# Florescence/UNet-Medical-Image-Contour-Segmentation

Hardware: NVIDIA B200
Metric: unet512_train_images_per_sec (higher is better)
Workload: dtype bf16

## Files before the change

### unet-medical-image-contour-segmentation_b200/csrc/common.cuh

```cuda
#pragma once
#include <cuda_bf16.h>
#include <cuda_runtime.h>
#include <stdint.h>
#include <stdio.h>

#include <string>

#include "../../include/unetb200.h"

namespace ub {

void set_error(const char* fmt, ...);
int cuda_fail(cudaError_t e, const char* what);

#define UB_CHECK_ARG(cond, ...)                \
  do {                                         \
    if (!(cond)) {                             \
      ub::set_error(__VA_ARGS__);              \
      return UNETB200_E_INVALID;               \
    }                                          \
  } while (0)

#define UB_LAUNCH_CHECK(what)                              \
  do {                                                     \
    cudaError_t e__ = cudaGetLastError();                  \
    if (e__ != cudaSuccess) return ub::cuda_fail(e__, what); \
  } while (0)

int sm_count();
int set_max_dynamic_smem(const void* func, int bytes, const char* what);

template <typename T>
struct Elem;
template <>
struct Elem<float> {
  static __device__ __forceinline__ float ld(const float* p) { return *p; }
  static __device__ __forceinline__ void st(float* p, float v) { *p = v; }
// ... 20 lines not shown
    v[2 * i + 1] = __uint_as_float(w[i] & 0xffff0000u);
  }
}
__device__ __forceinline__ uint32_t pack_bf16x2(float lo, float hi) {
  __nv_bfloat162 t = __floats2bfloat162_rn(lo, hi);
  return *reinterpret_cast<uint32_t*>(&t);
}
__device__ __forceinline__ void store8(float* p, const float v[8]) {
  *reinterpret_cast<float4*>(p) = make_float4(v[0], v[1], v[2], v[3]);
  *reinterpret_cast<float4*>(p + 4) = make_float4(v[4], v[5], v[6], v[7]);
}
__device__ __forceinline__ void store8(__nv_bfloat16* p, const float v[8]) {
  uint4 r;
  r.x = pack_bf16x2(v[0], v[1]);
  r.y = pack_bf16x2(v[2], v[3]);
  r.z = pack_bf16x2(v[4], v[5]);
  r.w = pack_bf16x2(v[6], v[7]);
  *reinterpret_cast<uint4*>(p) = r;
}

__device__ __forceinline__ float warp_sum(float v) {
#pragma unroll
  for (int o = 16; o > 0; o >>= 1) v += __shfl_xor_sync(0xffffffffu, v, o);
  return v;
}
__device__ __forceinline__ double warp_sum(double v) {
#pragma unroll
  for (int o = 16; o > 0; o >>= 1) v += __shfl_xor_sync(0xffffffffu, v, o);
  return v;
}

inline bool aligned16(const void* p) { return (reinterpret_cast<uintptr_t>(p) & 15) == 0; }

}
```

### unet-medical-image-contour-segmentation_b200/csrc/conv_first.cu

```cuda
#include "gconv.cuh"

namespace ub {

__device__ __forceinline__ void first_decode(const GconvDev& d, int m, int& b, int& i, int& j) {
  j = m % d.Wm;
  const int r = m / d.Wm;
  i = r % d.Hm;
  b = r / d.Hm;
}

template <typename T, int CIN>
__global__ void __launch_bounds__(256)
first_conv_fprop_kernel(GconvDev d, const T* __restrict__ x, const T* __restrict__ wp, T* __restrict__ y,
                        float* __restrict__ stats_ws) {
  constexpr int K = 9 * CIN;
  __shared__ float sstat[2][256];
  __shared__ float sw[CIN == 1 ? 1 : K * 256];
  const int G = d.N >> 3, lanes = 256 / G;
  const int g = threadIdx.x % G, lane = threadIdx.x / G;
  const bool active = lane < lanes;
  for (int i = threadIdx.x; i < 2 * 256; i += 256) (&sstat[0][0])[i] = 0.f;
  float wr[CIN == 1 ? K : 1][8];
  if constexpr (CIN == 1) {
#pragma unroll
// ... 300 lines not shown
      for (int c = 0; c < 3; ++c) { win[0][c] = win[1][c]; win[1][c] = win[2][c]; }
    }
  }
  if (stats_ws) {
    __shared__ float wstat[8][2][64];
    const int warp = threadIdx.x >> 5;
#pragma unroll
    for (int i = 0; i < 8; ++i) {
      float a = s[i], c = q[i];
      a += __shfl_xor_sync(0xffffffffu, a, 8); a += __shfl_xor_sync(0xffffffffu, a, 16);
      c += __shfl_xor_sync(0xffffffffu, c, 8); c += __shfl_xor_sync(0xffffffffu, c, 16);
      if ((threadIdx.x & 31) < 8) { wstat[warp][0][g * 8 + i] = a; wstat[warp][1][g * 8 + i] = c; }
    }
    __syncthreads();
    if (threadIdx.x < 128) {
      const int which = threadIdx.x >> 6, c = threadIdx.x & 63;
      float v = 0.f;
#pragma unroll
      for (int w = 0; w < 8; ++w) v += wstat[w][which][c];
      stats_ws[((long long)blockIdx.x * 2 + which) * 64 + c] = v;
    }
  }
}

template <typename T>
__device__ __forceinline__ float first_halo_elem(const GconvDev& d, const T* __restrict__ x, int b, int i0, int j0, int e) {
  const int r = e / (kFT_W + 2), c = e - r * (kFT_W + 2);
  const int gi = i0 - 1 + r, gj = j0 - 1 + c;
  if (e < (kFT_H + 2) * (kFT_W + 2) && (unsigned)gi < (unsigned)d.Hin && (unsigned)gj < (unsigned)d.Win)
    return Elem<T>::ld(x + ((long long)(b * d.Hin + gi) * d.Win + gj) * d.ld_in);
  return 0.f;
}

template <typename T>
__global__ void __launch_bounds__(256, 2)
first_conv_wgrad_tiled_kernel(GconvDev d, const T* __restrict__ x, const T* __restrict__ gy, float* __restrict__ partials,
                              int tiles_w, int tiles_h, int ntiles) {
  __shared__ float halo[kFT_H + 2][kFT_LD];
  const int g = threadIdx.x & 7, pl = threadIdx.x >> 3;
  float acc[3][3][8];
#pragma unroll
  for (int a = 0; a < 3; ++a)
#pragma unroll
    for (int c = 0; c < 3; ++c)
#pragma unroll
      for (int i = 0; i < 8; ++i) acc[a][c][i] = 0.f;
  auto decode = [&](int tile, int& b, int& i0, int& j0) {
    const int tj = tile % tiles_w;
    const int rest = tile / tiles_w;
    b = rest / tiles_h;
    i0 = (rest % tiles_h) * kFT_H;
    j0 = tj * kFT_W;
  };
  struct Row { uint4 a, b; };
  auto load_half = [&](int tile, int half, Row* dst) {
    int b, i0, j0;
    decode(tile, b, i0, j0);
    const int j = j0 + pl;
#pragma unroll
    for (int rr = 0; rr < 4; ++rr) {
      const int i = i0 + half * 4 + rr;
      dst[rr].a = make_uint4(0u, 0u, 0u, 0u);
      dst[rr].b = make_uint4(0u, 0u, 0u, 0u);
      if (tile < ntiles && i < d.Hm && j < d.Wm) {
        const T* src = gy + ((long long)(b * d.Hm + i) * d.Wm + j) * d.ld_out + g * 8;
        dst[rr].a = *reinterpret_cast<const uint4*>(src);
        if constexpr (sizeof(T) == 4) dst[rr].b = *reinterpret_cast<const uint4*>(src + 4);
// ... 2 lines not shown
  };
  auto unpack = [&](const Row& r, float v[8]) {
    if constexpr (sizeof(T) == 4) {
      v[0] = __uint_as_float(r.a.x); v[1] = __uint_as_float(r.a.y); v[2] = __uint_as_float(r.a.z); v[3] = __uint_as_float(r.a.w);
      v[4] = __uint_as_float(r.b.x); v[5] = __uint_as_float(r.b.y); v[6] = __uint_as_float(r.b.z); v[7] = __uint_as_float(r.b.w);
    } else {
      const uint32_t w[4] = {r.a.x, r.a.y, r.a.z, r.a.w};
#pragma unroll
      for (int i = 0; i < 4; ++i) { v[2 * i] = __uint_as_float(w[i] << 16); v[2 * i + 1] = __uint_as_float(w[i] & 0xffff0000u); }
    }
  };
  int tile = blockIdx.x;
  float h0 = 0.f, h1 = 0.f;
  Row cur[4], nxt[4];
  if (tile < ntiles) {
    int b, i0, j0;
    decode(tile, b, i0, j0);
    h0 = first_halo_elem<T>(d, x, b, i0, j0, threadIdx.x);
    h1 = first_halo_elem<T>(d, x, b, i0, j0, threadIdx.x + 256);
  }
  load_half(tile, 0, cur);
  for (; tile < ntiles; tile += gridDim.x) {
    __syncthreads();
    (&halo[0][0])[(threadIdx.x / (kFT_W + 2)) * kFT_LD + threadIdx.x % (kFT_W + 2)] = h0;
    if (threadIdx.x + 256 < (kFT_H + 2) * (kFT_W + 2))
      (&halo[0][0])[((threadIdx.x + 256) / (kFT_W + 2)) * kFT_LD + (threadIdx.x + 256) % (kFT_W + 2)] = h1;
    __syncthreads();
    const int nxt_tile = tile + gridDim.x;
    if (nxt_tile < ntiles) {
      int nb, ni0, nj0;
      decode(nxt_tile, nb, ni0, nj0);
      h0 = first_halo_elem<T>(d, x, nb, ni0, nj0, threadIdx.x);
      h1 = first_halo_elem<T>(d, x, nb, ni0, nj0, threadIdx.x + 256);
    }
    float win[3][3];
#pragma unroll
    for (int a = 0; a < 2; ++a)
#pragma unroll
      for (int c = 0; c < 3; ++c) win[a][c] = halo[a][pl + c];
#pragma unroll
    for (int half = 0; half < 2; ++half) {
      if (half == 0) load_half(tile, 1, nxt); else load_half(nxt_tile, 0, nxt);
#pragma unroll
      for (int rr = 0; rr < 4; ++rr) {
        const int r = half * 4 + rr;
        float gv[8];
        unpack(cur[rr], gv);
#pragma unroll
        for (int c = 0; c < 3; ++c) win[2][c] = halo[r + 2][pl + c];
#pragma unroll
        for (int a = 0; a < 3; ++a)
#pragma unroll
          for (int c = 0; c < 3; ++c)
#pragma unroll
            for (int k = 0; k < 8; ++k) acc[a][c][k] = fmaf(win[a][c], gv[k], acc[a][c][k]);
#pragma unroll
        for (int c = 0; c < 3; ++c) { win[0][c] = win[1][c]; win[1][c] = win[2][c]; }
      }
#pragma unroll
      for (int rr = 0; rr < 4; ++rr) cur[rr] = nxt[rr];
    }
  }
  __syncthreads();
  __shared__ int tmap[9];
  __shared__ float wred[8][9 * 64];
  if (threadIdx.x < 9) tmap[(d.tap_dy[threadIdx.x] + 1) * 3 + d.tap_dx[threadIdx.x] + 1] = threadIdx.x;
// ... 117 lines not shown
      default: GO(__nv_bfloat16, 4); break;
    }
  } else {
    switch (d->Cin) {
      case 1: GO(float, 1); break;
      case 2: GO(float, 2); break;
      case 3: GO(float, 3); break;
      default: GO(float, 4); break;
    }
  }
#undef GO
  cudaError_t e = cudaGetLastError();
  if (e != cudaSuccess) return cuda_fail(e, "first_conv_fprop");
  if (stats) return launch_stats_reduce(stats_ws, blocks, 2 * d->N, stats, s);
  return 0;
}

int first_wgrad_supported(const unetb200_gconv_t* d, const void* gy) {
  if (!first_common(d) || d->Cin != 1 || d->N > 128) return 0;
  const int G = d->N / 8;
  if (G & (G - 1)) return 0;
  return (!gy || aligned16(gy)) ? 1 : 0;
}

int first_wgrad_splits(const unetb200_gconv_t* d) {
  return first_blocks((long long)d->B * d->Hm * d->Wm, 256 / (d->N / 8));
}

int first_wgrad(const unetb200_gconv_t* d, const GconvDev& g, const void* x, const void* gy, float* partials,
                int splits, cudaStream_t s) {
  if (first_tiled_ok(d)) {
    const int tiles_w = (d->Wm + kFT_W - 1) / kFT_W, tiles_h = (d->Hm + kFT_H - 1) / kFT_H;
    const int ntiles = d->B * tiles_w * tiles_h;
    if (d->dtype == UNETB200_BF16)
      first_conv_wgrad_tiled_kernel<__nv_bfloat16><<<splits, 256, 0, s>>>(g, (const __nv_bfloat16*)x, (const __nv_bfloat16*)gy,
                                                                          partials, tiles_w, tiles_h, ntiles);
    else
      first_conv_wgrad_tiled_kernel<float><<<splits, 256, 0, s>>>(g, (const float*)x, (const float*)gy, partials, tiles_w,
                                                                  tiles_h, ntiles);
    cudaError_t e = cudaGetLastError();
    if (e != cudaSuccess) return cuda_fail(e, "first_conv_wgrad_tiled");
    return 0;
  }
  if (d->dtype == UNETB200_BF16)
    first_conv_wgrad_kernel<__nv_bfloat16><<<splits, 256, 0, s>>>(g, (const __nv_bfloat16*)x,
                                                                  (const __nv_bfloat16*)gy, partials);
  else
    first_conv_wgrad_kernel<float><<<splits, 256, 0, s>>>(g, (const float*)x, (const float*)gy, partials);
  cudaError_t e = cudaGetLastError();
  if (e != cudaSuccess) return cuda_fail(e, "first_conv_wgrad");
  return 0;
}

}
```

### unet-medical-image-contour-segmentation_b200/csrc/conv_tc3.cu

```cuda
#include <cstring>

#include "tc_common.cuh"

namespace ub {

__device__ __forceinline__ uint32_t cluster_ctarank() {
  uint32_t r;
  asm volatile("mov.u32 %0, %%cluster_ctarank;" : "=r"(r));
  return r;
}
__device__ __forceinline__ void cluster_sync_all() {
  asm volatile("barrier.cluster.arrive.release.aligned;\n\tbarrier.cluster.wait.acquire.aligned;" ::: "memory");
}
__device__ __forceinline__ uint32_t mapa_u32(uint32_t saddr, uint32_t rank) {
  uint32_t r;
  asm volatile("mapa.shared::cluster.u32 %0, %1, %2;" : "=r"(r) : "r"(saddr), "r"(rank));
  return r;
}
__device__ __forceinline__ void mbar_arrive_cluster(uint32_t cluster_addr) {
  asm volatile("mbarrier.arrive.release.cluster.shared::cluster.b64 _, [%0];" ::"r"(cluster_addr) : "memory");
}
__device__ __forceinline__ void mbar_arrive_local(uint64_t* bar) {
  asm volatile("mbarrier.arrive.shared::cta.b64 _, [%0];" ::"r"(smem_u32(bar)) : "memory");
}
// ... 85 lines not shown
        "=r"(v[25]), "=r"(v[26]), "=r"(v[27]), "=r"(v[28]), "=r"(v[29]), "=r"(v[30]), "=r"(v[31])
      : "r"(taddr)
      : "memory");
}
__device__ __forceinline__ uint32_t lds_u32(uint32_t saddr) {
  uint32_t v;
  asm volatile("ld.shared.u32 %0, [%1];" : "=r"(v) : "r"(saddr) : "memory");
  return v;
}
__device__ __forceinline__ void sts_v4(uint32_t saddr, uint32_t a, uint32_t b, uint32_t c, uint32_t d) {
  asm volatile("st.shared.v4.u32 [%0], {%1, %2, %3, %4};" ::"r"(saddr), "r"(a), "r"(b), "r"(c), "r"(d) : "memory");
}
__device__ __forceinline__ void tmem_ld_fence() { asm volatile("tcgen05.wait::ld.sync.aligned;" ::: "memory"); }
__device__ __forceinline__ void tma_store_wait_read_all() { asm volatile("cp.async.bulk.wait_group.read 0;" ::: "memory"); }

struct alignas(64) Tc3Params {
  CUtensorMap a_map;
  CUtensorMap b_map;
  CUtensorMap o_map;
  uint32_t tap_aoff[9];
  uint32_t a_box_bytes;
  uint32_t sub1_off;
  uint32_t row_bytes;
  int cchunks, Cin;
  int tiles_w, tiles_h, tile_w, tile_h;
  int sub1_di, sub1_dj;
  int m_tiles, m_groups, total_groups;
  int Hm, Wm, B;
  float* stats_ws;
  const float* affine;
  int N;
  CUtensorMap y_map;
  const float* bnc;
  const float* oc_w;
  const float* oc_b;
  void* logits;
  int ncls;
  void* pooled;
  long long ld_pool;
};

constexpr uint32_t kA3Stage = 44032;
constexpr int kEpi3Stage = 4096;
constexpr int kEpi3Warps = 8;
constexpr int kTc3Threads = 64 + 32 * kEpi3Warps;

constexpr int EPI_PLAIN = 0, EPI_AFFINE = 1, EPI_BNBWD = 2, EPI_AFFINE_OUT = 3;
template <typename T, int BLOCK_N, int SA, int SB, int ACC, int CG, int TPS, int EPI = EPI_PLAIN>
__global__ void __launch_bounds__(kTc3Threads, 1) tc3_conv_kernel(const __grid_constant__ Tc3Params p) {
  constexpr bool OUTC = EPI == EPI_AFFINE_OUT, AFFINE = EPI == EPI_AFFINE || OUTC, BNBWD = EPI == EPI_BNBWD;
  static_assert(!OUTC || (BLOCK_N == 64 && sizeof(T) == 2), "the OutConv epilogue is the bf16 N = 64 kernel");
  constexpr bool TF32 = sizeof(T) == 4;
  constexpr int EPR = 128 / sizeof(T);
  constexpr uint32_t kBTap = (BLOCK_N / CG) * 128;
  constexpr uint32_t kBStage = TPS * kBTap;
  static_assert(9 % TPS == 0, "taps per stage");
  constexpr int NCB = BLOCK_N / EPR;
  static_assert(2 * BLOCK_N * ACC <= 512, "TMEM columns");
  extern __shared__ uint8_t smem_raw[];
  uint8_t* smem = reinterpret_cast<uint8_t*>((reinterpret_cast<uintptr_t>(smem_raw) + 1023) & ~(uintptr_t)1023);
  uint8_t* a_ring = smem;
  uint8_t* b_ring = a_ring + SA * kA3Stage;
  uint8_t* epi = b_ring + SB * kBStage;
  uint8_t* yst = epi + kEpi3Warps * kEpi3Stage;
  uint64_t* bars = reinterpret_cast<uint64_t*>(yst + (BNBWD ? kEpi3Warps * kEpi3Stage : 0));
  uint64_t* a_full = bars;
  uint64_t* a_empty = a_full + SA;
  uint64_t* b_full = a_empty + SA;
  uint64_t* b_empty = b_full + SB;
  uint64_t* t_full = b_empty + SB;
  uint64_t* t_empty = t_full + ACC;
  uint64_t* y_full = t_empty + ACC;
  uint32_t* tmem_slot = reinterpret_cast<uint32_t*>(y_full + kEpi3Warps);

  const int warp = threadIdx.x >> 5, lane = threadIdx.x & 31;
  const uint32_t rank = CG == 2 ? cluster_ctarank() : 0u;
  const int group0 = blockIdx.x / CG, ngroups = gridDim.x / CG;
  if (warp == 0 && lane == 0) {
    tma_prefetch_desc(&p.a_map);
    tma_prefetch_desc(&p.b_map);
    tma_prefetch_desc(&p.o_map);
    for (int s = 0; s < SA; ++s) { mbar_init(&a_full[s], 1); mbar_init(&a_empty[s], 1); }
    for (int s = 0; s < SB; ++s) { mbar_init(&b_full[s], 1); mbar_init(&b_empty[s], 1); }
    for (int s = 0; s < ACC; ++s) { mbar_init(&t_full[s], 1); mbar_init(&t_empty[s], kEpi3Warps * CG); }
    if constexpr (BNBWD) {
      tma_prefetch_desc(&p.y_map);
      for (int s = 0; s < kEpi3Warps; ++s) mbar_init(&y_full[s], 1);
    }
    fence_barrier_init();
  }
  if (warp == 1) tmem_alloc_cg<CG>(tmem_slot, 512);
  if constexpr (OUTC) {
    float* ocs = reinterpret_cast<float*>(epi);
    for (int i = threadIdx.x; i < 64 * 8 + 8; i += blockDim.x) {
      const int c = i >> 3, k = i & 7;
      float v = 0.f;
      if (k < p.ncls) v = c < 64 ? __ldg(p.oc_w + k * 64 + c) : (p.oc_b ? __ldg(p.oc_b + k) : 0.f);
      ocs[i] = __bfloat162float(__float2bfloat16_rn(v));
    }
  }
  tc_fence_before();
  __syncthreads();
  if constexpr (CG == 2) cluster_sync_all();
  tc_fence_after();
  const uint32_t tmem_base = *tmem_slot;

  if (warp == 0) {
    uint32_t sa = 0, pa = 1, sb = 0, pb = 1;
    for (int gt = group0; gt < p.total_groups; gt += ngroups) {
      const int nb = gt / p.m_groups;
      int mt = (gt - nb * p.m_groups) * CG + (int)rank;
      const bool valid = mt < p.m_tiles;
      const int tj = mt % p.tiles_w;
      mt /= p.tiles_w;
      const int ti = mt % p.tiles_h;
      const int b = valid ? mt / p.tiles_h : p.B;
      const int i0 = ti * p.tile_h - 1, j0 = tj * p.tile_w - 1;
      const int n0 = nb * BLOCK_N + (int)rank * (BLOCK_N / CG);
      for (int c = 0; c < p.cchunks; ++c) {
        mbar_wait(&a_empty[sa], pa);
        if (elect_one()) {
          if (rank == 0) mbar_expect_tx(&a_full[sa], CG * p.a_box_bytes);
          tma_load_4d_cg<CG>(a_ring + sa * kA3Stage, &p.a_map, mapa_u32(smem_u32(&a_full[sa]), 0), c * EPR, j0, i0, b);
        }
        if (++sa == SA) { sa = 0; pa ^= 1; }
        for (int t = 0; t < 9; t += TPS) {
          mbar_wait(&b_empty[sb], pb);
          if (elect_one()) {
            if (rank == 0) mbar_expect_tx(&b_full[sb], CG * kBStage);
            const uint32_t bar = mapa_u32(smem_u32(&b_full[sb]), 0);
#pragma unroll
            for (int j = 0; j < TPS; ++j)
              tma_load_2d_cg<CG>(b_ring + sb * kBStage + j * kBTap, &p.b_map, bar, (t + j) * p.Cin + c * EPR, n0);
          }
          if (++sb == SB) { sb = 0; pb ^= 1; }
        }
      }
    }
  } else if (warp == 1) {
    if (rank == 0) {
      constexpr uint32_t idesc = make_idesc(TF32, false, false, 128 * CG, BLOCK_N);
      const uint64_t a_desc_t = make_desc(smem_u32(a_ring), 16, p.row_bytes);
      const uint64_t b_desc_t = make_desc(smem_u32(b_ring), 16, 1024);
      const uint32_t sub1 = p.sub1_off;
      uint32_t sa = 0, pa = 0, sb = 0, pb = 0, acc = 0, pacc = 1;
      for (int gt = group0; gt < p.total_groups; gt += ngroups) {
        mbar_wait(&t_empty[acc], pacc);
        tc_fence_after();
        const uint32_t d_tmem = tmem_base + acc * 2 * BLOCK_N;
        uint32_t accum = 0;
        for (int c = 0; c < p.cchunks; ++c) {
          mbar_wait(&a_full[sa], pa);
          const uint64_t a_desc0 = a_desc_t + sa * (kA3Stage >> 4);
          for (int t = 0; t < 9; t += TPS) {
            mbar_wait(&b_full[sb], pb);
            tc_fence_after();
            const uint64_t b_desc0 = b_desc_t + sb * (kBStage >> 4);
            if (elect_one()) {
#pragma unroll
              for (int j = 0; j < TPS; ++j) {
                const uint64_t a_desc1 = a_desc0 + p.tap_aoff[t + j];
                const uint64_t b_desc1 = b_desc0 + j * (kBTap >> 4);
#pragma unroll
                for (int kk = 0; kk < 4; ++kk) {
                  const uint32_t on = accum | (uint32_t)(j | kk);
                  umma_cg<CG, TF32>(d_tmem, a_desc1 + 2 * kk, b_desc1 + 2 * kk, idesc, on);
                  umma_cg<CG, TF32>(d_tmem + BLOCK_N, a_desc1 + sub1 + 2 * kk, b_desc1 + 2 * kk, idesc, on);
                }
              }
              umma_commit_cg<CG>(&b_empty[sb]);
              if (t + TPS == 9) umma_commit_cg<CG>(&a_empty[sa]);
            }
            __syncwarp();
            accum = 1;
            if (++sb == SB) { sb = 0; pb ^= 1; }
          }
          if (++sa == SA) { sa = 0; pa ^= 1; }
        }
        if (elect_one()) umma_commit_cg<CG>(&t_full[acc]);
        __syncwarp();
        if (++acc == ACC) { acc = 0; pacc ^= 1; }
      }
    }
  } else {
    const int quad = warp & 3;
    const int s = (warp - 2) >> 2;
    const int ew = s * 4 + quad;
    uint8_t* buf = epi + ew * kEpi3Stage;
    const uint32_t buf_s = smem_u32(buf);
    uint32_t acc = 0, pacc = 0;
    int cur_nb = -1;
    float st[NCB][TF32 ? 2 : 4];
#pragma unroll
    for (int i = 0; i < NCB; ++i)
#pragma unroll
      for (int j = 0; j < (TF32 ? 2 : 4); ++j) st[i][j] = 0.f;
    auto flush = [&](int nb) {
      if (!p.stats_ws || nb < 0) return;
      float* dst = p.stats_ws + (((long long)nb * gridDim.x + blockIdx.x) * kEpi3Warps + ew) * 2 * BLOCK_N;
#pragma unroll
      for (int cb = 0; cb < NCB; ++cb) {
        if constexpr (TF32) {
          dst[cb * 32 + lane] = st[cb][0];
          dst[BLOCK_N + cb * 32 + lane] = st[cb][1];
          st[cb][0] = st[cb][1] = 0.f;
        } else {
          dst[cb * 64 + 2 * lane] = st[cb][0];
          dst[BLOCK_N + cb * 64 + 2 * lane] = st[cb][1];
          dst[cb * 64 + 2 * lane + 1] = st[cb][2];
          dst[BLOCK_N + cb * 64 + 2 * lane + 1] = st[cb][3];
          st[cb][0] = st[cb][1] = st[cb][2] = st[cb][3] = 0.f;
        }
      }
    };
    const uint32_t t_empty_leader0 = mapa_u32(smem_u32(&t_empty[0]), 0);
    constexpr int CPL = TF32 ? 1 : 2;
    float bmu[BNBWD ? NCB : 1][CPL], bis[BNBWD ? NCB : 1][CPL], bsc[BNBWD ? NCB : 1][CPL], bsh[BNBWD ? NCB : 1][CPL];
    uint8_t* ybuf = yst + ew * kEpi3Stage;
    const uint32_t ybuf_s = smem_u32(ybuf);
    uint32_t yph = 0;
    auto y_fetch = [&](int gt2, int cb2) {
      const int nb2 = gt2 / p.m_groups;
      int mt2 = (gt2 - nb2 * p.m_groups) * CG + (int)rank;
      const bool valid2 = mt2 < p.m_tiles;
      const int tj2 = mt2 % p.tiles_w;
      mt2 /= p.tiles_w;
      const int ti2 = mt2 % p.tiles_h;
      const int b2 = valid2 ? mt2 / p.tiles_h : p.B;
      mbar_expect_tx(&y_full[ew], kEpi3Stage);
      tma_load_4d(ybuf, &p.y_map, &y_full[ew], nb2 * BLOCK_N + cb2 * EPR, tj2 * p.tile_w + s * p.sub1_dj,
                  ti2 * p.tile_h + s * p.sub1_di + 4 * quad, b2);
    };
    if constexpr (BNBWD) {
      if (lane == 0 && group0 < p.total_groups) y_fetch(group0, 0);
    }
    for (int gt = group0; gt < p.total_groups; gt += ngroups) {
      const int nb = gt / p.m_groups;
      int mt = (gt - nb * p.m_groups) * CG + (int)rank;
      const bool valid = mt < p.m_tiles;
      const int tj = mt % p.tiles_w;
      mt /= p.tiles_w;
      const int ti = mt % p.tiles_h;
      const int b = mt / p.tiles_h;
      const int n0 = nb * BLOCK_N;
      if (nb != cur_nb) {
        flush(cur_nb);
        cur_nb = nb;
        if constexpr (BNBWD) {
#pragma unroll
          for (int cb = 0; cb < NCB; ++cb)
#pragma unroll
            for (int k = 0; k < CPL; ++k) {
              const int ch = n0 + cb * EPR + CPL * lane + k;
              bmu[cb][k] = __ldg(p.bnc + ch);
              bis[cb][k] = __ldg(p.bnc + p.N + ch);
              bsc[cb][k] = __ldg(p.bnc + 2 * p.N + ch);
              bsh[cb][k] = __ldg(p.bnc + 3 * p.N + ch);
            }
        }
      }
      const int pi0 = ti * p.tile_h + s * p.sub1_di + 4 * quad;
      const int pj0 = tj * p.tile_w + s * p.sub1_dj;
      const uint32_t valid_rows =
          __ballot_sync(0xffffffffu, valid && (pi0 + (lane >> 3) < p.Hm) && (pj0 + (lane & 7) < p.Wm));
      mbar_wait(&t_full[acc], pacc);
      tc_fence_after();
// ... 64 lines not shown
              }
            }
          }
          fence_async_smem();
          __syncwarp();
          if (lane == 0) {
            tma_store_4d(&p.o_map, buf, n0 + cb * EPR, pj0, pi0, b);
            tma_store_commit();
          }
          if constexpr (AFFINE && !OUTC && !TF32) {
            if (p.pooled) {
              const int Hp = p.Hm >> 1, Wp = p.Wm >> 1;
              const int gy0 = pi0 >> 1, gx0 = pj0 >> 1;
#pragma unroll
              for (int py = 0; py < 2; ++py)
#pragma unroll
                for (int px = 0; px < 4; ++px) {
                  const int r0 = 16 * py + 2 * px;
                  uint32_t m = 0u;
#pragma unroll
                  for (int k = 0; k < 4; ++k) {
                    const int r = r0 + (k & 1) + 8 * (k >> 1);
                    m = __vmaxu2(m, lds_u32(buf_s + r * 128 + ((((lane >> 2) ^ (r & 7)) << 4) | ((lane & 3) << 2))));
                  }
                  if (valid && gy0 + py < Hp && gx0 + px < Wp)
                    reinterpret_cast<uint32_t*>(reinterpret_cast<__nv_bfloat16*>(p.pooled) +
                                                (((long long)b * Hp + gy0 + py) * Wp + gx0 + px) * p.ld_pool + n0 + cb * EPR)[lane] = m;
                }
            }
          }
          if constexpr (BNBWD) {
            float s0 = 0.f, q0 = 0.f, s1 = 0.f, q1 = 0.f;
            uint32_t u[32], yv[32];
            mbar_wait(&y_full[ew], yph);
            yph ^= 1;
#pragma unroll
            for (int r = 0; r < 32; ++r) {
              const uint32_t off = r * 128 + ((((lane >> 2) ^ (r & 7)) << 4) | ((lane & 3) << 2));
              u[r] = lds_u32(buf_s + off);
              yv[r] = lds_u32(ybuf_s + off);
            }
            __syncwarp();
            if (lane == 0) {
              if (cb + 1 < NCB) y_fetch(gt, cb + 1);
              else if (gt + ngroups < p.total_groups) y_fetch(gt + ngroups, 0);
            }
#pragma unroll
            for (int r = 0; r < 32; ++r) {
              const bool live = (valid_rows >> r) & 1u;
              if constexpr (TF32) {
                const float yy = __uint_as_float(yv[r]);
                const float gg = (live && fmaf(yy, bsc[cb][0], bsh[cb][0]) > 0.f) ? __uint_as_float(u[r]) : 0.f;
                s0 += gg; q0 += gg * ((yy - bmu[cb][0]) * bis[cb][0]);
              } else {
                const float ya = __uint_as_float(yv[r] << 16), yb = __uint_as_float(yv[r] & 0xffff0000u);
                const float ga = (live && fmaf(ya, bsc[cb][0], bsh[cb][0]) > 0.f) ? __uint_as_float(u[r] << 16) : 0.f;
                const float gb = (live && fmaf(yb, bsc[cb][1], bsh[cb][1]) > 0.f) ? __uint_as_float(u[r] & 0xffff0000u) : 0.f;
                s0 += ga; q0 += ga * ((ya - bmu[cb][0]) * bis[cb][0]);
                s1 += gb; q1 += gb * ((yb - bmu[cb][1]) * bis[cb][1]);
              }
            }
            st[cb][0] += s0; st[cb][1] += q0;
            if constexpr (!TF32) { st[cb][2] += s1; st[cb][3] += q1; }
          } else if (p.stats_ws) {
            float s0 = 0.f, q0 = 0.f, s1 = 0.f, q1 = 0.f;
            uint32_t u[32];
#pragma unroll
            for (int r = 0; r < 32; ++r)
              u[r] = lds_u32(buf_s + r * 128 + ((((lane >> 2) ^ (r & 7)) << 4) | ((lane & 3) << 2)));
            if (valid_rows == 0xffffffffu) {
#pragma unroll
              for (int r = 0; r < 32; ++r) {
                if constexpr (TF32) {
                  const float a = __uint_as_float(u[r]);
                  s0 += a; q0 = fmaf(a, a, q0);
                } else {
                  const float a = __uint_as_float(u[r] << 16), c2 = __uint_as_float(u[r] & 0xffff0000u);
                  s0 += a; q0 = fmaf(a, a, q0); s1 += c2; q1 = fmaf(c2, c2, q1);
                }
              }
            } else {
#pragma unroll
              for (int r = 0; r < 32; ++r) {
                const float m = ((valid_rows >> r) & 1u) ? 1.f : 0.f;
                if constexpr (TF32) {
                  const float a = __uint_as_float(u[r]) * m;
                  s0 += a; q0 = fmaf(a, a, q0);
                } else {
                  const float a = __uint_as_float(u[r] << 16) * m, c2 = __uint_as_float(u[r] & 0xffff0000u) * m;
                  s0 += a; q0 = fmaf(a, a, q0); s1 += c2; q1 = fmaf(c2, c2, q1);
                }
              }
            }
            st[cb][0] += s0; st[cb][1] += q0;
            if constexpr (!TF32) { st[cb][2] += s1; st[cb][3] += q1; }
          }
        }
      }
      if constexpr (BNBWD) {
        if (valid_rows == 0u) {
#pragma unroll 1
          for (int cb = 0; cb < NCB; ++cb) {
            mbar_wait(&y_full[ew], yph);
            yph ^= 1;
            __syncwarp();
            if (lane == 0) {
              if (cb + 1 < NCB) y_fetch(gt, cb + 1);
              else if (gt + ngroups < p.total_groups) y_fetch(gt + ngroups, 0);
            }
          }
        }
      }
      tc_fence_before();
      __syncwarp();
      if (lane == 0) {
        if constexpr (CG == 2) mbar_arrive_cluster(t_empty_leader0 + acc * 8);
        else mbar_arrive_local(&t_empty[acc]);
      }
      if (++acc == ACC) { acc = 0; pacc ^= 1; }
    }
    flush(cur_nb);
    if (lane == 0) tma_store_wait_all();
  }
  tc_fence_before();
  __syncthreads();
  if constexpr (CG == 2) cluster_sync_all();
  if (warp == 1) {
    __syncwarp();
    tmem_dealloc_cg<CG>(tmem_base, 512);
  }
}

// ... 25 lines not shown
  pl->CG = tc3_cluster_size();
  static const int max_bn = getenv("UNETB200_TC3_MAXBN") ? atoi(getenv("UNETB200_TC3_MAXBN")) : 128;
  pl->BN = (d->dtype == UNETB200_BF16 && d->N % 256 == 0 && max_bn >= 256) ? 256 : (d->N % 128 == 0 ? 128 : 64);
  if (d->Wm > 8) { pl->tile_w = 16; pl->tile_h = 16; }
  else { pl->tile_w = 8; pl->tile_h = 32; }
  pl->box_w = pl->tile_w + 2;
  pl->box_h = pl->tile_h + 2;
  const int tiles_w = (d->Wm + pl->tile_w - 1) / pl->tile_w, tiles_h = (d->Hm + pl->tile_h - 1) / pl->tile_h;
  pl->m_tiles = d->B * tiles_w * tiles_h;
  pl->m_groups = (pl->m_tiles + pl->CG - 1) / pl->CG;
  pl->n_blocks = d->N / pl->BN;
  const long long total = (long long)pl->m_groups * pl->n_blocks;
  const int slots = sm_count() / pl->CG;
  pl->grid = (int)(total < slots ? total : slots) * pl->CG;
  return true;
}

int tc3_fprop_supported(const unetb200_gconv_t* d, const void* x, const void* wp, const float* bias, const void* y) {
  static const bool off = getenv("UNETB200_NO_TC3") != nullptr;
  if (off || bias) return 0;
  if (d->dtype == UNETB200_F32 && d->algo != UNETB200_ALGO_TC && d->algo != UNETB200_ALGO_PREFER_TC) return 0;
  Tc3Plan pl;
  if (!tc3_plan(d, &pl)) return 0;
  if (!aligned16(x) || !aligned16(wp) || !aligned16(y)) return 0;
  return 1;
}

long long tc3_stats_workspace(const unetb200_gconv_t* d) {
  Tc3Plan pl;
  if (!tc3_plan(d, &pl)) return 0;
  return (long long)pl.n_blocks * pl.grid * kEpi3Warps * 2 * pl.BN;
}

template <typename T, int BN, int SA, int SB, int ACC, int CG, int TPS, int EPI = EPI_PLAIN>
static int tc3_launch(const Tc3Params& P, int grid, cudaStream_t s) {
  constexpr int smem = SA * kA3Stage + SB * TPS * (BN / CG) * 128 + (EPI == EPI_BNBWD ? 2 : 1) * kEpi3Warps * kEpi3Stage + 1024 + 256;
  static_assert(smem <= 227 * 1024, "shared memory budget");
  if (int rc = set_max_dynamic_smem(reinterpret_cast<const void*>(&tc3_conv_kernel<T, BN, SA, SB, ACC, CG, TPS, EPI>), smem,
                                    "tc3_conv smem attribute"))
    return rc;
  cudaLaunchConfig_t cfg = {};
  cfg.gridDim = dim3((unsigned)grid);
  cfg.blockDim = dim3(kTc3Threads);
  cfg.dynamicSmemBytes = smem;
  cfg.stream = s;
  cudaLaunchAttribute at[1];
  at[0].id = cudaLaunchAttributeClusterDimension;
  at[0].val.clusterDim.x = CG;
  at[0].val.clusterDim.y = 1;
  at[0].val.clusterDim.z = 1;
  cfg.attrs = at;
  cfg.numAttrs = 1;
  cudaError_t e = cudaLaunchKernelEx(&cfg, tc3_conv_kernel<T, BN, SA, SB, ACC, CG, TPS, EPI>, P);
  if (e != cudaSuccess) return cuda_fail(e, "tc3_conv launch");
  return 0;
}

__global__ void __launch_bounds__(1024) tc3_stats_reduce_kernel(const float* __restrict__ ws, int rows, int BN, int N, double* __restrict__ stats) {
  __shared__ double red[32][33];
  const int lane = threadIdx.x & 31, ry = threadIdx.x >> 5;
  const int nb = blockIdx.y;
  const int col = blockIdx.x * 32 + lane;
  double acc = 0.0;
  if (col < 2 * BN) {
    const float* base = ws + (long long)nb * rows * 2 * BN + col;
    int r = ry;
    for (; r + 96 < rows; r += 128) {
      const float a = base[(long long)r * 2 * BN], b = base[(long long)(r + 32) * 2 * BN],
                  c = base[(long long)(r + 64) * 2 * BN], d = base[(long long)(r + 96) * 2 * BN];
      acc += (double)a; acc += (double)b; acc += (double)c; acc += (double)d;
    }
    for (; r < rows; r += 32) acc += (double)base[(long long)r * 2 * BN];
  }
  red[ry][lane] = acc;
  __syncthreads();
  if (ry == 0 && col < 2 * BN) {
    double s = 0.0;
#pragma unroll
    for (int i = 0; i < 32; ++i) s += red[i][lane];
    const int which = col / BN, c = col - which * BN;
    stats[which * N + nb * BN + c] += s;
  }
}

int tc3_bnbwd_supported(const unetb200_gconv_t* d) {
  Tc3Plan pl;
// ... 25 lines not shown
    return UNETB200_E_INVALID;
  }
  if (!tc3_plan(d, &pl)) { set_error("tc3_fprop: unsupported shape"); return UNETB200_E_INVALID; }
  const int esz = d->dtype == UNETB200_BF16 ? 2 : 4;
  Tc3Params P;
  memset(&P, 0, sizeof(P));
  int rc = encode_act_box(&P.a_map, d->dtype, x, d->Cin, d->Win, d->Hin, d->B, d->ld_in, (long long)d->Win * d->ld_in,
                          (long long)d->Hin * d->Win * d->ld_in, pl.box_w, pl.box_h, false);
  if (rc) return rc;
  const char* obase = (const char*)y + ((long long)d->out_off_y * d->Wout + d->out_off_x) * d->ld_out * (long long)esz;
  rc = encode_act_box(&P.o_map, d->dtype, obase, d->N, d->Wm, d->Hm, d->B, d->ld_out, (long long)d->Wout * d->ld_out,
                      (long long)d->Hout * d->Wout * d->ld_out, 8, 4, false);
  if (rc) return rc;
  rc = encode_weights(&P.b_map, d->dtype, wp, g.K, d->N, pl.BN / pl.CG);
  if (rc) return rc;
  for (int t = 0; t < 9; ++t)
    P.tap_aoff[t] = (uint32_t)(((d->tap_dy[t] + 1) * pl.box_w + (d->tap_dx[t] + 1)) * 128) >> 4;
  P.a_box_bytes = (uint32_t)(pl.box_w * pl.box_h * 128);
  P.row_bytes = (uint32_t)pl.box_w * 128;
  if (pl.tile_w == 16) { P.sub1_di = 0; P.sub1_dj = 8; P.sub1_off = (8 * 128) >> 4; }
  else { P.sub1_di = 16; P.sub1_dj = 0; P.sub1_off = (uint32_t)(16 * pl.box_w * 128) >> 4; }
  P.cchunks = d->Cin / (128 / esz);
  P.Cin = d->Cin;
  P.tile_w = pl.tile_w; P.tile_h = pl.tile_h;
  P.tiles_w = (d->Wm + pl.tile_w - 1) / pl.tile_w;
  P.tiles_h = (d->Hm + pl.tile_h - 1) / pl.tile_h;
  P.m_tiles = pl.m_tiles; P.m_groups = pl.m_groups;
  P.total_groups = pl.m_groups * pl.n_blocks;
  P.Hm = d->Hm; P.Wm = d->Wm; P.B = d->B;
  P.stats_ws = stats ? stats_ws : nullptr;
  P.affine = affine;
  P.N = d->N;
  P.bnc = bnc;
  P.pooled = pooled; P.ld_pool = ld_pool;
  if (yprev) {
    rc = encode_act_box(&P.y_map, d->dtype, yprev, d->N, d->Wm, d->Hm, d->B, ld_yprev, (long long)d->Wm * ld_yprev,
                        (long long)d->Hm * d->Wm * ld_yprev, 8, 4, false);
    if (rc) return rc;
  }
  if (oc) {
    if (!affine || !tc3_affine_outconv_supported(d, oc->ncls) || !oc->w || !oc->logits) {
      set_error("tc3_fprop: the OutConv epilogue needs the folded BatchNorm coefficients, bf16, N = 64 and n_classes <= 8");
      return UNETB200_E_INVALID;
    }
    P.oc_w = oc->w; P.oc_b = oc->b; P.logits = oc->logits; P.ncls = oc->ncls;
    return tc3_launch<__nv_bfloat16, 64, 3, 3, 2, 2, 3, EPI_AFFINE_OUT>(P, pl.grid, stream);
  }
  if (affine) {
    if (pl.BN == 256) { set_error("tc3_fprop: affine epilogue supports N blocks of 64 / 128"); return UNETB200_E_INVALID; }
    if (d->dtype == UNETB200_BF16) {
      if (pl.CG == 2) return pl.BN == 128 ? tc3_launch<__nv_bfloat16, 128, 2, 3, 2, 2, 3, EPI_AFFINE>(P, pl.grid, stream)
                                          : tc3_launch<__nv_bfloat16, 64, 3, 3, 2, 2, 3, EPI_AFFINE>(P, pl.grid, stream);
      return pl.BN == 128 ? tc3_launch<__nv_bfloat16, 128, 2, 6, 2, 1, 1, EPI_AFFINE>(P, pl.grid, stream)
                          : tc3_launch<__nv_bfloat16, 64, 3, 6, 2, 1, 1, EPI_AFFINE>(P, pl.grid, stream);
    }
    if (pl.CG == 2) return pl.BN == 128 ? tc3_launch<float, 128, 2, 3, 2, 2, 3, EPI_AFFINE>(P, pl.grid, stream)
                                        : tc3_launch<float, 64, 3, 3, 2, 2, 3, EPI_AFFINE>(P, pl.grid, stream);
    return pl.BN == 128 ? tc3_launch<float, 128, 2, 6, 2, 1, 1, EPI_AFFINE>(P, pl.grid, stream)
                        : tc3_launch<float, 64, 3, 6, 2, 1, 1, EPI_AFFINE>(P, pl.grid, stream);
  }
  if (stats) {
    cudaError_t e = cudaMemsetAsync(stats_ws, 0, sizeof(float) * (size_t)tc3_stats_workspace(d), stream);
    if (e != cudaSuccess) return cuda_fail(e, "tc3 stats workspace memset");
  }
  if (yprev) {
    if (pl.CG != 2 || pl.BN == 256) { set_error("tc3_fprop: BatchNorm-backward epilogue: CTA pairs, N blocks of 64 / 128"); return UNETB200_E_INVALID; }
    static const int cfg64 = getenv("UNETB200_BNBWD64_CFG") ? atoi(getenv("UNETB200_BNBWD64_CFG")) : 1;
    if (d->dtype == UNETB200_BF16)
      rc = pl.BN == 128 ? tc3_launch<__nv_bfloat16, 128, 2, 3, 2, 2, 3, EPI_BNBWD>(P, pl.grid, stream)
           : cfg64 == 1 ? tc3_launch<__nv_bfloat16, 64, 3, 2, 2, 2, 3, EPI_BNBWD>(P, pl.grid, stream)
                        : tc3_launch<__nv_bfloat16, 64, 2, 3, 2, 2, 3, EPI_BNBWD>(P, pl.grid, stream);
    else
      rc = pl.BN == 128 ? tc3_launch<float, 128, 2, 3, 2, 2, 3, EPI_BNBWD>(P, pl.grid, stream)
                        : tc3_launch<float, 64, 3, 2, 2, 2, 3, EPI_BNBWD>(P, pl.grid, stream);
  } else if (d->dtype == UNETB200_BF16) {
    if (pl.CG == 2) {
      if (pl.BN == 256) rc = tc3_launch<__nv_bfloat16, 256, 2, 2, 1, 2, 3>(P, pl.grid, stream);
      else if (pl.BN == 128) rc = tc3_launch<__nv_bfloat16, 128, 2, 3, 2, 2, 3>(P, pl.grid, stream);
      else rc = tc3_launch<__nv_bfloat16, 64, 3, 3, 2, 2, 3>(P, pl.grid, stream);
    } else {
      if (pl.BN == 256) rc = tc3_launch<__nv_bfloat16, 256, 2, 3, 1, 1, 1>(P, pl.grid, stream);
      else if (pl.BN == 128) rc = tc3_launch<__nv_bfloat16, 128, 2, 6, 2, 1, 1>(P, pl.grid, stream);
      else rc = tc3_launch<__nv_bfloat16, 64, 3, 6, 2, 1, 1>(P, pl.grid, stream);
    }
  } else {
    if (pl.CG == 2) {
      if (pl.BN == 128) rc = tc3_launch<float, 128, 2, 3, 2, 2, 3>(P, pl.grid, stream);
      else rc = tc3_launch<float, 64, 3, 3, 2, 2, 3>(P, pl.grid, stream);
    } else {
      if (pl.BN == 128) rc = tc3_launch<float, 128, 2, 6, 2, 1, 1>(P, pl.grid, stream);
      else rc = tc3_launch<float, 64, 3, 6, 2, 1, 1>(P, pl.grid, stream);
    }
  }
  if (rc) return rc;
  if (stats) {
    const int rows = pl.grid * kEpi3Warps;
    tc3_stats_reduce_kernel<<<dim3((2 * pl.BN + 31) / 32, pl.n_blocks), 1024, 0, stream>>>(stats_ws, rows, pl.BN, d->N, stats);
    cudaError_t e = cudaGetLastError();
    if (e != cudaSuccess) return cuda_fail(e, "tc3_stats_reduce");
  }
  return 0;
}


// ... 236 lines not shown
```

Baseline: 711.5.

## Keep dgrad weights resident in smem and load BN-bwd y via registers

```diff
diff --git a/unet-medical-image-contour-segmentation_b200/csrc/common.cuh b/unet-medical-image-contour-segmentation_b200/csrc/common.cuh
--- a/unet-medical-image-contour-segmentation_b200/csrc/common.cuh
+++ b/unet-medical-image-contour-segmentation_b200/csrc/common.cuh
@@ -3,6 +3,7 @@
 #include <cuda_runtime.h>
 #include <stdint.h>
 #include <stdio.h>
+#include <stdlib.h>
 
 #include <string>
 
@@ -89,4 +90,9 @@
 
 inline bool aligned16(const void* p) { return (reinterpret_cast<uintptr_t>(p) & 15) == 0; }
 
+inline bool fullres_v0() {
+  static const bool v0 = getenv("UNETB200_FULLRES_V0") != nullptr;
+  return v0;
 }
+
+}
diff --git a/unet-medical-image-contour-segmentation_b200/csrc/conv_first.cu b/unet-medical-image-contour-segmentation_b200/csrc/conv_first.cu
--- a/unet-medical-image-contour-segmentation_b200/csrc/conv_first.cu
+++ b/unet-medical-image-contour-segmentation_b200/csrc/conv_first.cu
@@ -356,7 +356,7 @@
   return 0.f;
 }
 
-template <typename T>
+template <typename T, bool L2PF>
 __global__ void __launch_bounds__(256, 2)
 first_conv_wgrad_tiled_kernel(GconvDev d, const T* __restrict__ x, const T* __restrict__ gy, float* __restrict__ partials,
                               int tiles_w, int tiles_h, int ntiles) {
@@ -425,6 +425,14 @@
       decode(nxt_tile, nb, ni0, nj0);
       h0 = first_halo_elem<T>(d, x, nb, ni0, nj0, threadIdx.x);
       h1 = first_halo_elem<T>(d, x, nb, ni0, nj0, threadIdx.x + 256);
+      if constexpr (L2PF) {
+        const int i = ni0 + g, j = nj0 + pl;
+        if (i < d.Hm && j < d.Wm) {
+          const char* row = reinterpret_cast<const char*>(gy + ((long long)(nb * d.Hm + i) * d.Wm + j) * d.ld_out);
+#pragma unroll
+          for (int o = 0; o < 64 * (int)sizeof(T); o += 128) asm volatile("prefetch.global.L2 [%0];" ::"l"(row + o));
+        }
+      }
     }
     float win[3][3];
 #pragma unroll
@@ -608,12 +616,15 @@
   if (first_tiled_ok(d)) {
     const int tiles_w = (d->Wm + kFT_W - 1) / kFT_W, tiles_h = (d->Hm + kFT_H - 1) / kFT_H;
     const int ntiles = d->B * tiles_w * tiles_h;
-    if (d->dtype == UNETB200_BF16)
-      first_conv_wgrad_tiled_kernel<__nv_bfloat16><<<splits, 256, 0, s>>>(g, (const __nv_bfloat16*)x, (const __nv_bfloat16*)gy,
-                                                                          partials, tiles_w, tiles_h, ntiles);
-    else
-      first_conv_wgrad_tiled_kernel<float><<<splits, 256, 0, s>>>(g, (const float*)x, (const float*)gy, partials, tiles_w,
-                                                                  tiles_h, ntiles);
+    const bool pf = !fullres_v0();
+#define GOW(T, PF) \
+  first_conv_wgrad_tiled_kernel<T, PF><<<splits, 256, 0, s>>>(g, (const T*)x, (const T*)gy, partials, tiles_w, tiles_h, ntiles)
+    if (d->dtype == UNETB200_BF16) {
+      if (pf) GOW(__nv_bfloat16, true); else GOW(__nv_bfloat16, false);
+    } else {
+      if (pf) GOW(float, true); else GOW(float, false);
+    }
+#undef GOW
     cudaError_t e = cudaGetLastError();
     if (e != cudaSuccess) return cuda_fail(e, "first_conv_wgrad_tiled");
     return 0;
diff --git a/unet-medical-image-contour-segmentation_b200/csrc/conv_tc3.cu b/unet-medical-image-contour-segmentation_b200/csrc/conv_tc3.cu
--- a/unet-medical-image-contour-segmentation_b200/csrc/conv_tc3.cu
+++ b/unet-medical-image-contour-segmentation_b200/csrc/conv_tc3.cu
@@ -141,6 +141,8 @@
   int N;
   CUtensorMap y_map;
   const float* bnc;
+  const uint32_t* yprev;
+  long long ld_y32;
   const float* oc_w;
   const float* oc_b;
   void* logits;
@@ -150,12 +152,13 @@
 };
 
 constexpr uint32_t kA3Stage = 44032;
+constexpr uint32_t kA3Stage16 = 41984;
 constexpr int kEpi3Stage = 4096;
 constexpr int kEpi3Warps = 8;
 constexpr int kTc3Threads = 64 + 32 * kEpi3Warps;
 
 constexpr int EPI_PLAIN = 0, EPI_AFFINE = 1, EPI_BNBWD = 2, EPI_AFFINE_OUT = 3;
-template <typename T, int BLOCK_N, int SA, int SB, int ACC, int CG, int TPS, int EPI = EPI_PLAIN>
+template <typename T, int BLOCK_N, int SA, int SB, int ACC, int CG, int TPS, int EPI = EPI_PLAIN, bool RESB = false>
 __global__ void __launch_bounds__(kTc3Threads, 1) tc3_conv_kernel(const __grid_constant__ Tc3Params p) {
   constexpr bool OUTC = EPI == EPI_AFFINE_OUT, AFFINE = EPI == EPI_AFFINE || OUTC, BNBWD = EPI == EPI_BNBWD;
   static_assert(!OUTC || (BLOCK_N == 64 && sizeof(T) == 2), "the OutConv epilogue is the bf16 N = 64 kernel");
@@ -166,10 +169,13 @@
   static_assert(9 % TPS == 0, "taps per stage");
   constexpr int NCB = BLOCK_N / EPR;
   static_assert(2 * BLOCK_N * ACC <= 512, "TMEM columns");
+  static_assert(!RESB || SB * TPS == 9, "resident weights: one B stage per group of taps");
+  static_assert(!RESB || (BNBWD && NCB == 1 && sizeof(T) == 2), "resident weights: the bf16 N = 64 BatchNorm-backward dgrad");
+  constexpr uint32_t kAS = RESB ? kA3Stage16 : kA3Stage;
   extern __shared__ uint8_t smem_raw[];
   uint8_t* smem = reinterpret_cast<uint8_t*>((reinterpret_cast<uintptr_t>(smem_raw) + 1023) & ~(uintptr_t)1023);
   uint8_t* a_ring = smem;
-  uint8_t* b_ring = a_ring + SA * kA3Stage;
+  uint8_t* b_ring = a_ring + SA * kAS;
   uint8_t* epi = b_ring + SB * kBStage;
   uint8_t* yst = epi + kEpi3Warps * kEpi3Stage;
   uint64_t* bars = reinterpret_cast<uint64_t*>(yst + (BNBWD ? kEpi3Warps * kEpi3Stage : 0));
@@ -230,10 +236,11 @@
         mbar_wait(&a_empty[sa], pa);
         if (elect_one()) {
           if (rank == 0) mbar_expect_tx(&a_full[sa], CG * p.a_box_bytes);
-          tma_load_4d_cg<CG>(a_ring + sa * kA3Stage, &p.a_map, mapa_u32(smem_u32(&a_full[sa]), 0), c * EPR, j0, i0, b);
+          tma_load_4d_cg<CG>(a_ring + sa * kAS, &p.a_map, mapa_u32(smem_u32(&a_full[sa]), 0), c * EPR, j0, i0, b);
         }
         if (++sa == SA) { sa = 0; pa ^= 1; }
         for (int t = 0; t < 9; t += TPS) {
+          if (RESB && gt != group0) break;
           mbar_wait(&b_empty[sb], pb);
           if (elect_one()) {
             if (rank == 0) mbar_expect_tx(&b_full[sb], CG * kBStage);
@@ -260,9 +267,9 @@
         uint32_t accum = 0;
         for (int c = 0; c < p.cchunks; ++c) {
           mbar_wait(&a_full[sa], pa);
-          const uint64_t a_desc0 = a_desc_t + sa * (kA3Stage >> 4);
+          const uint64_t a_desc0 = a_desc_t + sa * (kAS >> 4);
           for (int t = 0; t < 9; t += TPS) {
-            mbar_wait(&b_full[sb], pb);
+            if (!RESB || gt == group0) mbar_wait(&b_full[sb], pb);
             tc_fence_after();
             const uint64_t b_desc0 = b_desc_t + sb * (kBStage >> 4);
             if (elect_one()) {
@@ -277,7 +284,7 @@
                   umma_cg<CG, TF32>(d_tmem + BLOCK_N, a_desc1 + sub1 + 2 * kk, b_desc1 + 2 * kk, idesc, on);
                 }
               }
-              umma_commit_cg<CG>(&b_empty[sb]);
+              if constexpr (!RESB) umma_commit_cg<CG>(&b_empty[sb]);
               if (t + TPS == 9) umma_commit_cg<CG>(&a_empty[sa]);
             }
             __syncwarp();
@@ -340,7 +347,24 @@
       tma_load_4d(ybuf, &p.y_map, &y_full[ew], nb2 * BLOCK_N + cb2 * EPR, tj2 * p.tile_w + s * p.sub1_dj,
                   ti2 * p.tile_h + s * p.sub1_di + 4 * quad, b2);
     };
-    if constexpr (BNBWD) {
+    uint32_t ynx[RESB ? 32 : 1];
+    auto y_load = [&](int gt2) {
+      int mt2 = gt2 * CG + (int)rank;
+      const bool valid2 = gt2 < p.total_groups && mt2 < p.m_tiles;
+      const int tj2 = mt2 % p.tiles_w;
+      mt2 /= p.tiles_w;
+      const int ti2 = mt2 % p.tiles_h;
+      const int b2 = mt2 / p.tiles_h;
+      const int qi = ti2 * p.tile_h + s * p.sub1_di + 4 * quad, qj = tj2 * p.tile_w + s * p.sub1_dj;
+#pragma unroll
+      for (int r = 0; r < 32; ++r) {
+        const int i = qi + (r >> 3), j = qj + (r & 7);
+        ynx[r] = (valid2 && i < p.Hm && j < p.Wm) ? __ldg(p.yprev + (((long long)b2 * p.Hm + i) * p.Wm + j) * p.ld_y32 + lane) : 0u;
+      }
+    };
+    if constexpr (RESB) {
+      y_load(group0);
+    } else if constexpr (BNBWD) {
       if (lane == 0 && group0 < p.total_groups) y_fetch(group0, 0);
     }
     for (int gt = group0; gt < p.total_groups; gt += ngroups) {
@@ -471,18 +495,27 @@
           if constexpr (BNBWD) {
             float s0 = 0.f, q0 = 0.f, s1 = 0.f, q1 = 0.f;
             uint32_t u[32], yv[32];
-            mbar_wait(&y_full[ew], yph);
-            yph ^= 1;
-#pragma unroll
-            for (int r = 0; r < 32; ++r) {
-              const uint32_t off = r * 128 + ((((lane >> 2) ^ (r & 7)) << 4) | ((lane & 3) << 2));
-              u[r] = lds_u32(buf_s + off);
-              yv[r] = lds_u32(ybuf_s + off);
-            }
-            __syncwarp();
-            if (lane == 0) {
-              if (cb + 1 < NCB) y_fetch(gt, cb + 1);
-              else if (gt + ngroups < p.total_groups) y_fetch(gt + ngroups, 0);
+            if constexpr (RESB) {
+#pragma unroll
+              for (int r = 0; r < 32; ++r) {
+                u[r] = lds_u32(buf_s + r * 128 + ((((lane >> 2) ^ (r & 7)) << 4) | ((lane & 3) << 2)));
+                yv[r] = ynx[r];
+              }
+              y_load(gt + ngroups);
+            } else {
+              mbar_wait(&y_full[ew], yph);
+              yph ^= 1;
+#pragma unroll
+              for (int r = 0; r < 32; ++r) {
+                const uint32_t off = r * 128 + ((((lane >> 2) ^ (r & 7)) << 4) | ((lane & 3) << 2));
+                u[r] = lds_u32(buf_s + off);
+                yv[r] = lds_u32(ybuf_s + off);
+              }
+              __syncwarp();
+              if (lane == 0) {
+                if (cb + 1 < NCB) y_fetch(gt, cb + 1);
+                else if (gt + ngroups < p.total_groups) y_fetch(gt + ngroups, 0);
+              }
             }
 #pragma unroll
             for (int r = 0; r < 32; ++r) {
@@ -536,7 +569,9 @@
           }
         }
       }
-      if constexpr (BNBWD) {
+      if constexpr (RESB) {
+        if (valid_rows == 0u) y_load(gt + ngroups);
+      } else if constexpr (BNBWD) {
         if (valid_rows == 0u) {
 #pragma unroll 1
           for (int cb = 0; cb < NCB; ++cb) {
@@ -628,11 +663,11 @@
   return (long long)pl.n_blocks * pl.grid * kEpi3Warps * 2 * pl.BN;
 }
 
-template <typename T, int BN, int SA, int SB, int ACC, int CG, int TPS, int EPI = EPI_PLAIN>
+template <typename T, int BN, int SA, int SB, int ACC, int CG, int TPS, int EPI = EPI_PLAIN, bool RESB = false>
 static int tc3_launch(const Tc3Params& P, int grid, cudaStream_t s) {
-  constexpr int smem = SA * kA3Stage + SB * TPS * (BN / CG) * 128 + (EPI == EPI_BNBWD ? 2 : 1) * kEpi3Warps * kEpi3Stage + 1024 + 256;
+  constexpr int smem = SA * (RESB ? kA3Stage16 : kA3Stage) + SB * TPS * (BN / CG) * 128 + (EPI == EPI_BNBWD ? 2 : 1) * kEpi3Warps * kEpi3Stage + 1024 + 256;
   static_assert(smem <= 227 * 1024, "shared memory budget");
-  if (int rc = set_max_dynamic_smem(reinterpret_cast<const void*>(&tc3_conv_kernel<T, BN, SA, SB, ACC, CG, TPS, EPI>), smem,
+  if (int rc = set_max_dynamic_smem(reinterpret_cast<const void*>(&tc3_conv_kernel<T, BN, SA, SB, ACC, CG, TPS, EPI, RESB>), smem,
                                     "tc3_conv smem attribute"))
     return rc;
   cudaLaunchConfig_t cfg = {};
@@ -647,7 +682,7 @@
   at[0].val.clusterDim.z = 1;
   cfg.attrs = at;
   cfg.numAttrs = 1;
-  cudaError_t e = cudaLaunchKernelEx(&cfg, tc3_conv_kernel<T, BN, SA, SB, ACC, CG, TPS, EPI>, P);
+  cudaError_t e = cudaLaunchKernelEx(&cfg, tc3_conv_kernel<T, BN, SA, SB, ACC, CG, TPS, EPI, RESB>, P);
   if (e != cudaSuccess) return cuda_fail(e, "tc3_conv launch");
   return 0;
 }
@@ -739,6 +774,8 @@
   P.affine = affine;
   P.N = d->N;
   P.bnc = bnc;
+  P.yprev = reinterpret_cast<const uint32_t*>(yprev);
+  P.ld_y32 = ld_yprev * (d->dtype == UNETB200_BF16 ? 2 : 4) / 4;
   P.pooled = pooled; P.ld_pool = ld_pool;
   if (yprev) {
     rc = encode_act_box(&P.y_map, d->dtype, yprev, d->N, d->Wm, d->Hm, d->B, ld_yprev, (long long)d->Wm * ld_yprev,
@@ -772,11 +809,15 @@
   }
   if (yprev) {
     if (pl.CG != 2 || pl.BN == 256) { set_error("tc3_fprop: BatchNorm-backward epilogue: CTA pairs, N blocks of 64 / 128"); return UNETB200_E_INVALID; }
-    static const int cfg64 = getenv("UNETB200_BNBWD64_CFG") ? atoi(getenv("UNETB200_BNBWD64_CFG")) : 1;
+    static const int cfg64 = getenv("UNETB200_BNBWD64_CFG") ? atoi(getenv("UNETB200_BNBWD64_CFG")) : (fullres_v0() ? 1 : 4);
+    const bool resb = P.cchunks == 1 && pl.n_blocks == 1 && P.a_box_bytes <= kA3Stage16;
     if (d->dtype == UNETB200_BF16)
       rc = pl.BN == 128 ? tc3_launch<__nv_bfloat16, 128, 2, 3, 2, 2, 3, EPI_BNBWD>(P, pl.grid, stream)
-           : cfg64 == 1 ? tc3_launch<__nv_bfloat16, 64, 3, 2, 2, 2, 3, EPI_BNBWD>(P, pl.grid, stream)
-                        : tc3_launch<__nv_bfloat16, 64, 2, 3, 2, 2, 3, EPI_BNBWD>(P, pl.grid, stream);
+           : (cfg64 == 4 && resb) ? tc3_launch<__nv_bfloat16, 64, 3, 3, 3, 2, 3, EPI_BNBWD, true>(P, pl.grid, stream)
+           : (cfg64 == 3 && resb) ? tc3_launch<__nv_bfloat16, 64, 3, 3, 2, 2, 3, EPI_BNBWD, true>(P, pl.grid, stream)
+           : cfg64 == 2 ? tc3_launch<__nv_bfloat16, 64, 3, 2, 3, 2, 3, EPI_BNBWD>(P, pl.grid, stream)
+           : cfg64 == 0 ? tc3_launch<__nv_bfloat16, 64, 2, 3, 2, 2, 3, EPI_BNBWD>(P, pl.grid, stream)
+                        : tc3_launch<__nv_bfloat16, 64, 3, 2, 2, 2, 3, EPI_BNBWD>(P, pl.grid, stream);
     else
       rc = pl.BN == 128 ? tc3_launch<float, 128, 2, 3, 2, 2, 3, EPI_BNBWD>(P, pl.grid, stream)
                         : tc3_launch<float, 64, 3, 2, 2, 2, 3, EPI_BNBWD>(P, pl.grid, stream);
```

New measurement: 701.5 (median of 6 runs). 0.986x the previous value.
